# SEU-dynamical-models/Manifold-based-optical-flow-method

Measured on AMD Instinct MI355X. Metric: flow timesteps/sec on 160k-vertex mesh, higher is better.
Workload: dtype f32

## Files before the change

include/mof.h:

```cpp
#ifndef MOF_H_
#define MOF_H_

#include <stdint.h>

#ifdef __cplusplus
extern "C" {
#endif

#define MOF_ABI_VERSION 4

#define MOF_OK 0
#define MOF_E_ARG (-1)
#define MOF_E_HIP (-2)
#define MOF_E_NOCONV (-3)
#define MOF_E_STATE (-4)

#define MOF_GEOM_F32_POINTS 1u
#define MOF_NO_REORDER 2u

#define MOF_PREC_F64 0
#define MOF_PREC_MIXED 1

#define MOF_IO_DEVICE 1u
#define MOF_NO_BLOCK_JACOBI 2u
// ... 136 lines not shown

int mof_residual_probe(const int32_t *tri, int32_t N, int32_t M, uint32_t flags, int64_t *staged_bytes,
                       int32_t *staged_used);
int mof_test_force_residual_rows(int32_t on);
int mof_test_force_residual_trips(int32_t on);
int mof_test_residual_launches(int64_t *counts);

int mof_assembly_probe(const int32_t *tri, int32_t N, int32_t M, uint32_t flags, int64_t *staged_bytes,
                       int32_t *staged_used);
int mof_test_force_assembly_rows(int32_t on);
int mof_test_force_assembly_trips(int32_t on);
int mof_test_assembly_launches(int64_t *counts);
int mof_test_assembly_readback(mof_mesh *mesh, int32_t system, float *A32, void *A0h, double *rhs,
                               int32_t *have_A0h);

int mof_xcd_map_check(int32_t nblk, int32_t batch, int32_t group);
int mof_xcd_batch_cap(int64_t nblk, int32_t group, int32_t *batch);

typedef struct mof_dd mof_dd;

typedef struct mof_dd_info {
    int32_t nparts;
    int32_t local_parts;
    int32_t rank;
    int32_t max_neighbours;
    int32_t max_owned;
    int32_t pad_;
    int64_t ghost_rows;
    int64_t send_rows;
    double ms_setup;
// ... 45 lines not shown
```

manifold-based-optical-flow-method_amd/csrc/mof_abi.cpp:

```cpp
#include <algorithm>
#include <chrono>
#include <cmath>
#include <cstring>
#include <cstdio>
#include <cstdlib>
#include <functional>
#include <future>
#include <memory>
#include <mutex>
#include <new>

#include "mof_amg.h"
#include "mof_dd.h"
#include "mof_hostio.h"
#include "mof_internal.h"

namespace {

thread_local std::string g_err;

template <class F>
int guarded(F &&f) {
    try {
        f();
// ... 338 lines not shown
}

}

int mof_io_guard(const std::function<void()> &f) { return guarded(f); }

namespace mof {

std::atomic<int> g_force_index32{0};
std::atomic<int> g_force_residual_rows{0};
std::atomic<int> g_force_residual_trips{0};
std::atomic<int64_t> g_residual_launches[3];
std::atomic<int> g_force_assembly_rows{0};
std::atomic<int> g_force_assembly_trips{0};
std::atomic<int64_t> g_assembly_launches[3];

void raise_lds_limit(LdsLimit &st, int device, std::initializer_list<const void *> kernels, int64_t cap) {
    MOF_REQUIRE(device >= 0 && device < LdsLimit::kMaxDev, "device index out of range");
    std::call_once(st.once[device], [&] {
        for (const void *k : kernels)
            MOF_HIP(hipFuncSetAttribute(k, hipFuncAttributeMaxDynamicSharedMemorySize, (int)cap));
    });
}

void mesh_set_own(mof_mesh *m, int32_t nown) {
    MOF_HIP(hipSetDevice(m->device));
    m->n_own = nown;
    const int sym = knob(Knob::SymReads) ? (knob_int(Knob::SymReads, 0) != 0) : -1;
    std::shared_ptr<const MirrorTable> mt;
    {
// ... 13 lines not shown
        }
    }
    m->sym_reads = mt->used;
    const std::vector<int32_t> &mir = mt->table;
    m->sell_mir.alloc(mir.size());
    m->sell_mir.upload(mir.data(), mir.size(), m->stream);
    m->idx_packed = !mt->packed.empty() && !g_force_index32.load();
    if (m->idx_packed) {
        m->sell_idx.alloc(mt->packed.size());
        m->sell_idx.upload(mt->packed.data(), mt->packed.size(), m->stream);
    }
    m->res_lds_bytes = res_staged_bytes(m->pat);
    m->res_lds = m->res_lds_bytes <= kResLdsCap && !g_force_residual_rows.load();
    m->asm_lds_bytes = asm_staged_bytes(m->pat);
    m->asm_lds = asm_staged_fits(m->pat) && !g_force_assembly_rows.load();
    int64_t own = 0;
    for (int32_t v : mir) own += v >= 0 && !(v & kMirT);
    m->blocks_read = own;
    MOF_HIP(hipStreamSynchronize(m->stream));
}

constexpr int32_t kRowsPerWindow = 256;

void mesh_prepare_host(mof_mesh *m, const double *xyz, const double *nrm, const int32_t *tri,
                       const double *area, int32_t N, int32_t M, uint32_t flags, const int32_t *perm_in,
                       const int32_t *tri_ids) {
    m->N = N;
    m->n_own = N;
    m->M = M;
    m->flags = flags;
// ... 784 lines not shown
        MOF_REQUIRE(system >= 0 && system < w.JB && w.A32.n >= 4 * nb * (b + 1) &&
                        w.rhs.n >= 2 * (size_t)m->N * (b + 1),
                    "no mixed-precision assembly of that system in the workspace");
        MOF_HIP(hipStreamSynchronize(m->stream));
        if (A32) MOF_HIP(hipMemcpy(A32, w.A32.p + 4 * nb * b, 4 * nb * sizeof(float), hipMemcpyDeviceToHost));
        if (rhs)
            MOF_HIP(hipMemcpy(rhs, w.rhs.p + 2 * (size_t)m->N * b, 2 * (size_t)m->N * sizeof(double),
                              hipMemcpyDeviceToHost));
        const void *h = m->amg ? mof::amg_fine(m).A0h : nullptr;
        if (have_A0h) *have_A0h = h != nullptr;
        if (A0h && h)
            MOF_HIP(hipMemcpy(A0h, static_cast<const uint2 *>(h) + nb * b, nb * sizeof(uint2), hipMemcpyDeviceToHost));
    });
}

int mof_xcd_map_check(int32_t nblk, int32_t batch, int32_t group) {
    return guarded([&] {
        MOF_REQUIRE(nblk > 0 && batch > 0 && group >= 0, "bad arguments");
        MOF_REQUIRE(mof::xcd_map_covers(nblk, batch, group), "XCD order does not cover every (row block, system) once");
    });
}

int mof_xcd_batch_cap(int64_t nblk, int32_t group, int32_t *batch) {
    return guarded([&] {
        MOF_REQUIRE(nblk > 0 && group >= 0 && batch, "bad arguments");
        *batch = mof::xcd_batch_cap_host(nblk, group);
    });
}

int mof_bench_spmv(mof_mesh *m, uint32_t precision, int32_t batch, int32_t reps,
// ... 12 lines not shown
```

manifold-based-optical-flow-method_amd/csrc/mof_amg.hip:

```cpp
#include <algorithm>
#include <cstdio>
#include <cstdlib>

#include "mof_amg.h"
#include "mof_rowkern.h"

namespace mof {
namespace {

constexpr int kB3 = 12;

__device__ __forceinline__ bool retired(const int32_t *sysi, int32_t b) {
    return !sysi[b * kSysStride + SI_ACTIVE] || sysi[b * kSysStride + SI_CONV] >= 0;
}

template <int BS>
__device__ __forceinline__ void ldv(const float *v, int64_t node, float (&x)[BS]) {
    if constexpr (BS == 2) {
        const float2 t = reinterpret_cast<const float2 *>(v)[node];
        x[0] = t.x; x[1] = t.y;
    } else {
        const float4 t = reinterpret_cast<const float4 *>(v)[node];
        x[0] = t.x; x[1] = t.y; x[2] = t.z;
    }
// ... 64 lines not shown

__device__ __forceinline__ void st3(float *A, int64_t idx, const float (&a)[3][3]) {
    float4 *p = reinterpret_cast<float4 *>(A) + 3 * idx;
#pragma unroll
    for (int r = 0; r < 3; ++r) p[r] = make_float4(a[r][0], a[r][1], a[r][2], 0.f);
}

__device__ __forceinline__ void st_h9(uint4 *H, uint16_t *H22, int64_t q, const float (&c)[3][3]) {
    H[q] = make_uint4(bf16_bits(c[0][0]) | (bf16_bits(c[0][1]) << 16), bf16_bits(c[0][2]) | (bf16_bits(c[1][0]) << 16),
                      bf16_bits(c[1][1]) | (bf16_bits(c[1][2]) << 16), bf16_bits(c[2][0]) | (bf16_bits(c[2][1]) << 16));
    H22[q] = (uint16_t)bf16_bits(c[2][2]);
}

constexpr size_t kAhWords = 2, kAh22Words = 2;

__device__ __forceinline__ void st_a9(uint4 *H, uint16_t *H22, int64_t q, const float (&c)[3][3]) {
    {
        float m = 0.f;
#pragma unroll
        for (int r = 0; r < 3; ++r)
#pragma unroll
            for (int k = 0; k < 3; ++k) m = fmaxf(m, fabsf(c[r][k]));
        const uint32_t sb = bf16_bits(m / 127.f);
        const float sc = bf16_lo(sb);
        uint32_t u[9];
#pragma unroll
        for (int r = 0; r < 3; ++r)
#pragma unroll
            for (int k = 0; k < 3; ++k) {
                const float v = sc > 0.f ? rintf(c[r][k] / sc) : 0.f;
                u[3 * r + k] = (uint32_t)(fminf(fmaxf(v, -127.f), 127.f) + 128.f);
            }
        reinterpret_cast<uint2 *>(H)[q] =
            make_uint2(u[0] | (u[1] << 8) | (u[2] << 16) | (u[3] << 24), u[4] | (u[5] << 8) | (u[6] << 16) | (u[7] << 24));
        reinterpret_cast<uint32_t *>(H22)[q] = u[8] | (sb << 16);
    }
}
__device__ __forceinline__ void st_pair(float *__restrict__ Ac, uint4 *__restrict__ Ah, uint16_t *__restrict__ Ah22,
                                        int64_t b, int64_t c_sell_nb, int64_t pos, int32_t tw,
                                        const float (&C)[3][3]) {
    st3(Ac, b * c_sell_nb + pos, C);
    if (Ah) st_a9(Ah, Ah22, b * c_sell_nb + pos, C);
    if (tw >= 0) {
        float T[3][3];
#pragma unroll
        for (int r = 0; r < 3; ++r)
#pragma unroll
            for (int c = 0; c < 3; ++c) T[r][c] = C[c][r];
        st3(Ac, b * c_sell_nb + tw, T);
        if (Ah) st_a9(Ah, Ah22, b * c_sell_nb + tw, T);
    }
}


__global__ __launch_bounds__(kWG) void k_to_h0(int64_t n, const float4 *__restrict__ A, uint2 *__restrict__ H) {
    const int64_t q = (int64_t)blockIdx.x * kWG + threadIdx.x;
    if (q >= n) return;
    const float4 v = A[q];
    h0_st(H, q, v.x, v.y, v.z, v.w);
}

constexpr int kGalNS = 4;
__global__ __launch_bounds__(kWG) void k_galerkin0_ns(
    int64_t c_sell_nb, int32_t nC, int32_t B, const int32_t *__restrict__ c_sell_row,
    const int32_t *__restrict__ c_diag, const uint8_t *__restrict__ c_dead, const int32_t *__restrict__ c_twin,
// ... 73 lines not shown
    }
#pragma unroll
    for (int t = 0; t < kGalNS; ++t) {
        const int32_t b = b0 + t;
        if (b >= B) continue;
        if (pos == c_diag[I]) {
#pragma unroll
            for (int d = 0; d < 3; ++d)
                if (c_dead[3 * (int64_t)I + d]) Cm[t][d][d] += 1.f;
            float D[3][3];
            inv3(Cm[t], D);
            st_h9(Dh, Dh22, (int64_t)b * nC + I, D);
        }
        st_pair(Ac, Ah, Ah22, b, c_sell_nb, pos, c_twin[pos], Cm[t]);
    }
}

constexpr int kGalENS = 2;
__global__ __launch_bounds__(kWG) void k_galerkin0_ent(
    int32_t ngrp, const int32_t *__restrict__ ggrp, int32_t nC, int32_t B, const int32_t *__restrict__ c_sell_row,
    const int32_t *__restrict__ c_diag, const uint8_t *__restrict__ c_dead, const int32_t *__restrict__ c_twin, const int32_t *__restrict__ gptr,
    const int32_t *__restrict__ gent, const float *__restrict__ Q, const uint2 *__restrict__ Afh,
    int64_t f_sell_nb, int64_t c_sell_nb, float *__restrict__ Ac, uint4 *__restrict__ Dh,
    uint16_t *__restrict__ Dh22, uint4 *__restrict__ Ah, uint16_t *__restrict__ Ah22) {
#pragma clang fp contract(off)
    __shared__ float con[kGalENS][9][kWG];
    int32_t g, bq;
    const int32_t nq = (B + kGalENS - 1) / kGalENS;
    if (!xcd_map(ngrp, nq, g, bq, kGrpGal)) return;
    const int32_t b0 = bq * kGalENS;
// ... 6 lines not shown
        const int32_t pos = p0 + (int32_t)threadIdx.x / kGalENS;
        tI = c_sell_row[pos];
        tq0 = gptr[pos];
        tq1 = gptr[pos + 1];
        if (tI < nC) tdg = c_diag[tI];
    }
    if (e < e1) {
        const int32_t fp = gent[3 * (int64_t)e], ii = gent[3 * (int64_t)e + 1], jj = gent[3 * (int64_t)e + 2];
        float qi[6], qj[6], a[kGalENS][4];
#pragma unroll
        for (int k = 0; k < 6; ++k) {
            qi[k] = Q[(int64_t)ii * 6 + k];
            qj[k] = Q[(int64_t)jj * 6 + k];
        }
        const int32_t fq = fp < 0 ? 0 : fp & kMirPos;
        const bool tr = fp >= 0 && (fp & kMirT);
#pragma unroll
        for (int t = 0; t < kGalENS; ++t) {
            const int64_t bb = min(b0 + t, B - 1);
            h0_dec(h0_ld(Afh, bb * f_sell_nb + fq), a[t][0], a[t][1], a[t][2], a[t][3]);
            if (tr) {
                const float t01 = a[t][1];
                a[t][1] = a[t][2];
                a[t][2] = t01;
            }
            if (fp < 0) {
                const float d = fp == -1 ? 1.f : 0.f;
                a[t][0] = d; a[t][1] = 0.f; a[t][2] = 0.f; a[t][3] = d;
            }
        }
#pragma unroll
        for (int t = 0; t < kGalENS; ++t) {
            float T[2][3];
#pragma unroll
            for (int r = 0; r < 2; ++r)
#pragma unroll
                for (int c = 0; c < 3; ++c) T[r][c] = 1.f * (a[t][2 * r] * qj[c] + a[t][2 * r + 1] * qj[3 + c]);
#pragma unroll
            for (int r = 0; r < 3; ++r)
#pragma unroll
                for (int c = 0; c < 3; ++c) con[t][3 * r + c][threadIdx.x] = qi[r] * T[0][c] + qi[3 + r] * T[1][c];
        }
    }
    __syncthreads();
    for (int32_t task = threadIdx.x; task < np * kGalENS; task += kWG) {
        const int32_t pos = p0 + task / kGalENS, t = task % kGalENS, b = b0 + t;
        const bool first = task == (int32_t)threadIdx.x;
        const int32_t I = first ? tI : c_sell_row[pos];
        if (I >= nC || b >= B) continue;
        float Cm[3][3] = {};
        const int32_t q0 = first ? tq0 : gptr[pos], q1 = first ? tq1 : gptr[pos + 1];
        const bool diag = pos == (first ? tdg : c_diag[I]);
        if (q0 == q1 && !diag) continue;
        for (int32_t q = q0; q < q1; ++q)
#pragma unroll
            for (int k = 0; k < 9; ++k) Cm[k / 3][k % 3] += con[t][k][q - e0];
        if (diag) {
#pragma unroll
            for (int d = 0; d < 3; ++d)
                if (c_dead[3 * (int64_t)I + d]) Cm[d][d] += 1.f;
            float D[3][3];
            inv3(Cm, D);
            st_h9(Dh, Dh22, (int64_t)b * nC + I, D);
        }
        st_pair(Ac, Ah, Ah22, b, c_sell_nb, pos, c_twin[pos], Cm);
    }
}

constexpr int kSlab = 64;
constexpr int kSlabPos = 64;
template <typename T>
__global__ __launch_bounds__(kWG) void k_a_slab(int64_t f_sell_nb, int32_t b0, int32_t nb,
                                                const T *__restrict__ Af, T *__restrict__ AI) {
    __shared__ T t[kSlabPos][kSlab + 1];
    const int64_t q0 = (int64_t)blockIdx.x * kSlabPos;
    const int32_t lane = (int32_t)threadIdx.x & 63, w = (int32_t)threadIdx.x >> 6;
    for (int32_t s = w; s < kSlab; s += kWG / 64) {
        const int64_t q = q0 + lane;
        T v = {};
        if (s < nb && q < f_sell_nb) v = Af[(int64_t)(b0 + s) * f_sell_nb + q];
// ... 1590 lines not shown
    G.bf16_fresh = true;
    return AmgBf16{reinterpret_cast<uint2 *>(G.A0h.p)};
}

AmgFine amg_fine(mof_mesh *m) {
    AmgDevice &G = *m->amg;
    AmgFine f;
    f.A0h = G.A0h.p;
    f.sell_nb = m->pat.sell_nb();
    f.sell_off = m->sell_off.p;
    f.x0 = G.lv[0].x.p;
    f.omega = G.omega;
    f.smoothed = G.lv[0].smoothed;
    f.regular = G.regular;
    return f;
}

static uint4 *ah(AmgDevLevel &C) { return C.Ah.n > 1 ? reinterpret_cast<uint4 *>(C.Ah.p) : nullptr; }
static uint16_t *ah22(AmgDevLevel &C) { return C.Ah22.n > 1 ? C.Ah22.p : nullptr; }
static uint4 *dh(AmgDevLevel &C) { return reinterpret_cast<uint4 *>(C.Dh.p); }

void amg_setup_batch(mof_mesh *m, int32_t B, hipStream_t s) {
    AmgDevice &G = *m->amg;
    Workspace &w = m->ws;
    const size_t L = G.lv.size();
    if (!G.bf16_fresh) {
        const int64_t nb0 = m->pat.sell_nb() * B;
        k_to_h0<<<dim3((unsigned)((nb0 + kWG - 1) / kWG)), kWG, 0, s>>>(
            nb0, reinterpret_cast<const float4 *>(w.A32.p), reinterpret_cast<uint2 *>(G.A0h.p));
    }
// ... 36 lines not shown
                k_galerkin_sys<2><<<sys_grid(C.sell_nb), kWG, 0, s>>>(
                    C.sell_nb, C.n, B, b0, C.sell_row.p, C.diag_pos.p, C.dead.p, C.twin.p, F.gptr.p, F.gent.p, F.Q.p,
                    reinterpret_cast<const float4 *>(G.aslab.p), C.A.p, dh(C), C.Dh22.p, ah(C), ah22(C), cs);
            if (l1) {
                AmgDevLevel &C2 = G.lv[2];
                k_galerkin_sys<3><<<sys_grid(C2.sell_nb), kWG, 0, s>>>(
                    C2.sell_nb, C2.n, B, b0, C2.sell_row.p, C2.diag_pos.p, C2.dead.p, C2.twin.p, C.gptr.p, C.gent.p, C.Q.p,
                    reinterpret_cast<const float4 *>(C.slab.p), C2.A.p, dh(C2), C2.Dh22.p, ah(C2), ah22(C2), nullptr);
            }
        }
        l_first = l1 ? 2 : 1;
    }
    for (size_t l = l_first; l + 1 < L; ++l) {
        AmgDevLevel &F = G.lv[l], &C = G.lv[l + 1];
        const bool ent = ent_fits(F);
        if (l == 0 && ent)
            k_galerkin0_ent<<<dim3(xcd_grid(F.nggrp, (B + kGalENS - 1) / kGalENS, kGrpGal)), kWG, 0, s>>>(
                F.nggrp, F.ggrp.p, C.n, B, C.sell_row.p, C.diag_pos.p, C.dead.p, C.twin.p, F.gptr.p, F.gent.p, F.Q.p,
                reinterpret_cast<const uint2 *>(G.A0h.p), m->pat.sell_nb(), C.sell_nb, C.A.p, dh(C), C.Dh22.p, ah(C),
                ah22(C));
        else if (l == 0)
            k_galerkin0_ns<<<dim3(xcd_grid((int32_t)((C.sell_nb + kWG - 1) / kWG), (B + kGalNS - 1) / kGalNS,
                                           kGrpGal)),
                             kWG, 0, s>>>(C.sell_nb, C.n, B, C.sell_row.p, C.diag_pos.p, C.dead.p, C.twin.p, F.gptr.p, F.gent.p,
                                          F.Q.p, w.A32.p, m->pat.sell_nb(), C.A.p, dh(C), C.Dh22.p, ah(C), ah22(C),
                                          F.smoothed ? nullptr : reinterpret_cast<const uint2 *>(G.A0h.p));
        else if (ent) {
            if (F.nggrp > 0)
                k_galerkin3_ent<<<dim3(xcd_grid(F.nggrp, (B + kGalENS - 1) / kGalENS, kGrpGal)), kWG, 0, s>>>(
                    F.nggrp, F.ggrp.p, C.n, B, C.sell_row.p, C.diag_pos.p, C.dead.p, C.twin.p, F.gptr.p, F.gent.p, F.Q.p, F.A.p,
                    F.sell_nb, C.sell_nb, C.A.p, dh(C), C.Dh22.p, ah(C), ah22(C));
            if (F.nbig > 0)
                k_galerkin3_big<kGalBigNS>
                    <<<dim3(xcd_grid(F.nbig, (B + kGalBigNS - 1) / kGalBigNS, kGrpGal)), kWG, 0, s>>>(
                        F.nbig, F.gbig.p, C.n, B, C.sell_row.p, C.diag_pos.p, C.dead.p, C.twin.p, F.gptr.p, F.gent.p, F.Q.p,
                        F.A.p, F.sell_nb, C.sell_nb, C.A.p, dh(C), C.Dh22.p, ah(C), ah22(C));
        } else
            k_galerkin3_ns<kGal3NS>
                <<<dim3(xcd_grid((int32_t)((C.sell_nb + kWG - 1) / kWG), (B + kGal3NS - 1) / kGal3NS, kGrpGal)), kWG,
                   0, s>>>(C.sell_nb, C.n, B, C.sell_row.p, C.diag_pos.p, C.dead.p, C.twin.p, F.gptr.p, F.gent.p, F.Q.p, F.A.p,
                           F.sell_nb, C.A.p, dh(C), C.Dh22.p, ah(C), ah22(C));
    }
// ... 155 lines not shown
```

manifold-based-optical-flow-method_amd/csrc/mof_internal.h:

```cpp
#pragma once

#include <hip/hip_runtime.h>

#include <atomic>
#include <cstdint>
#include <cstdlib>
#include <functional>
#include <future>
#include <initializer_list>
#include <memory>
#include <mutex>
#include <string>
#include <type_traits>
#include <vector>

#include "../../include/mof.h"
#include "mof_knobs.h"

namespace mof {

constexpr int kWG = 256;
constexpr int kSlice = 64;

struct Error {
// ... 83 lines not shown
extern std::atomic<int> g_force_residual_rows;
extern std::atomic<int> g_force_residual_trips;
extern std::atomic<int64_t> g_residual_launches[3];
constexpr int64_t kAsmLdsCap = 160 * 1024;
constexpr int32_t kAsmLdsMaxW = 8;
inline int64_t asm_slice_bytes(int32_t w_a2, int32_t w_inc) {
    return (int64_t)kSlice * ((int64_t)w_inc * 112 + (int64_t)w_a2 * 48 + 48);
}
int64_t asm_staged_bytes(const Pattern &pat);
inline bool asm_staged_fits(const Pattern &pat) {
    return pat.max_w <= kAsmLdsMaxW && asm_staged_bytes(pat) <= kAsmLdsCap;
}
extern std::atomic<int> g_force_assembly_rows;
extern std::atomic<int> g_force_assembly_trips;
extern std::atomic<int64_t> g_assembly_launches[3];

struct LdsLimit {
    static constexpr int kMaxDev = 64;
    std::once_flag once[kMaxDev];
};
void raise_lds_limit(LdsLimit &st, int device, std::initializer_list<const void *> kernels, int64_t cap);

struct Workspace {
    int32_t cap = 0;
    int32_t nblk = 0;
    DevArray<double> u64, fc;
    DevArray<float> u32;
    DevArray<float> A32;
    DevArray<double> A64;
    DevArray<double> dinv64;
// ... 69 lines not shown
    std::vector<int32_t> agg_order;
    mof::DevArray<int32_t> perm_d;
    mof::DevArray<int32_t> tri_orig;
    mof::DevArray<int32_t> icol;
    mof::DevArray<int32_t> tri, vptr, vcol, cptr, clist, sell_off, sell_col, sell_blk, blk_row,
        diag_pos, tsell_off, tinc, tslot;
    mof::DevArray<int32_t> sell_mir;
    int64_t blocks_read = 0;
    bool sym_reads = false;
    mof::DevArray<uint32_t> sell_idx;
    bool idx_packed = false;
    int64_t res_lds_bytes = 0;
    bool res_lds = false;
    int64_t asm_lds_bytes = 0;
    bool asm_lds = false;
    mof::DevArray<double> e, gw, iw, area, a2;
    mof::DevArray<double> a2s64, w12_64;
    mof::DevArray<float> a2s32, w12_32;
    double a2s_lambda = 0.0;
    bool a2s_valid = false;
    mof::DevArray<double> Aexp, fexp;
    mof::Workspace ws;
    bool have_last_A = false;
    double ms_geometry = 0.0, ms_pattern = 0.0;
    int32_t *h_sysi = nullptr;
    double *h_sysd = nullptr;
    int32_t h_cap = 0;
    std::vector<hipEvent_t> spmv_events;
    std::vector<int32_t> iter_hint;
    mof::AmgDevice *amg = nullptr;
// ... 82 lines not shown
bool amg_build(mof_mesh *m);
void amg_ensure(mof_mesh *m, int32_t B);
void amg_setup_batch(mof_mesh *m, int32_t B, hipStream_t s);
void amg_vcycle(mof_mesh *m, int32_t B, const float *r, float *z, double *part_slot, int32_t nblk,
                const RedArgs &rd, hipStream_t s, bool zh, const int32_t *smap = nullptr, int32_t nl = 0);
struct AmgFine {
    const void *A0h;
    int64_t sell_nb;
    const int32_t *sell_off;
    float *x0;
    float omega;
    bool smoothed;
    bool regular;
};
AmgFine amg_fine(mof_mesh *m);
struct AmgBf16 {
    uint2 *A0h;
};
AmgBf16 amg_bf16_targets(mof_mesh *m, int32_t B);
void amg_destroy(AmgDevice *g);

int32_t amg_levels(const mof_mesh *m);
float amg_set_omega(mof_mesh *m, float omega);

bool xcd_map_covers(int32_t nblk, int32_t B, int32_t grp);
int32_t xcd_batch_cap_host(int64_t nblk, int32_t grp);
double bench_spmv(mof_mesh *m, uint32_t precision, int32_t B, int32_t reps, hipStream_t s,
                  double *bytes);

}
// ... 1 lines not shown
```

manifold-based-optical-flow-method_amd/mofhip/_lib.py:

```python
from __future__ import annotations

import ctypes
import os
import subprocess
import threading

import numpy as np

PKG_DIR = os.path.dirname(os.path.abspath(__file__))
ROOT_DIR = os.path.dirname(PKG_DIR)
CSRC_DIR = os.path.join(ROOT_DIR, "csrc")
LIB_PATH = os.environ.get("MOFHIP_LIB") or os.path.join(PKG_DIR, "libmofhip.so")

MOF_ABI_VERSION = 4

MOF_OK = 0
MOF_E_ARG = -1
MOF_E_HIP = -2
MOF_E_NOCONV = -3
MOF_E_STATE = -4

MOF_GEOM_F32_POINTS = 1
MOF_NO_REORDER = 2
MOF_PREC_F64 = 0
# ... 14 lines not shown

EXPORTS = (
    "mof_version", "mof_abi_version", "mof_last_error", "mof_device_count", "mof_mesh_create", "mof_mesh_clone",
    "mof_mesh_destroy", "mof_mesh_get_info", "mof_geometry_export", "mof_csr_export",
    "mof_assemble", "mof_solve_range", "mof_bench_spmv", "mof_velocity_vectors",
    "mof_csv_write", "mof_csv_shape", "mof_csv_read", "mof_ply_info", "mof_ply_read",
    "mof_point_normals", "mof_cell_areas", "mof_singularities", "mof_amg_probe",
    "mof_partition_rcb", "mof_dd_plan_info", "mof_dd_create", "mof_dd_unique_id",
    "mof_dd_create_rank", "mof_dd_destroy", "mof_dd_get_info", "mof_dd_solve_range",
    "mof_dd_test_fail_recovery_alloc", "mof_mesh_prepare", "mof_mesh_sync",
    "mof_singularities_compact", "mof_xcd_map_check", "mof_xcd_batch_cap", "mof_dd_create_rank_host",
    "mof_index_probe", "mof_test_force_index32", "mof_wave_speed", "mof_streamline_map", "mof_streamlines",
    "mof_test_streamline_pass", "mof_residual_probe", "mof_test_force_residual_rows",
    "mof_test_force_residual_trips", "mof_test_residual_launches", "mof_assembly_probe",
    "mof_test_force_assembly_rows", "mof_test_force_assembly_trips", "mof_test_assembly_launches",
    "mof_test_assembly_readback",
)


class MofError(RuntimeError):

    def __init__(self, code, msg):
        super().__init__("libmofhip error %d: %s" % (code, msg))
        self.code = code


class NotConverged(MofError):
    pass


class MofOpts(ctypes.Structure):
# ... 108 lines not shown
            "mof_test_streamline_pass": ([i32], ctypes.c_int),
            "mof_singularities": ([i32, P, P, i32, i32, P, i32, f64, u32, P, P, P, P, P],
                                  ctypes.c_int),
            "mof_amg_probe": ([P, P, i32, i32, P, P, P, P], ctypes.c_int),
            "mof_index_probe": ([P, i32, i32, u32, i32, P, P, P, P, P, P, P], ctypes.c_int),
            "mof_test_force_index32": ([i32], ctypes.c_int),
            "mof_residual_probe": ([P, i32, i32, u32, P, P], ctypes.c_int),
            "mof_test_force_residual_rows": ([i32], ctypes.c_int),
            "mof_test_force_residual_trips": ([i32], ctypes.c_int),
            "mof_test_residual_launches": ([P], ctypes.c_int),
            "mof_assembly_probe": ([P, i32, i32, u32, P, P], ctypes.c_int),
            "mof_test_force_assembly_rows": ([i32], ctypes.c_int),
            "mof_test_force_assembly_trips": ([i32], ctypes.c_int),
            "mof_test_assembly_launches": ([P], ctypes.c_int),
            "mof_test_assembly_readback": ([P, i32, P, P, P, P], ctypes.c_int),
            "mof_xcd_map_check": ([i32, i32, i32], ctypes.c_int),
            "mof_xcd_batch_cap": ([i64, i32, P], ctypes.c_int),
            "mof_singularities_compact": ([i32, P, P, i32, i32, P, i32, f64, u32, P, i64, P, P, P, P, P,
                                           P, P], ctypes.c_int),
            "mof_partition_rcb": ([P, i32, i32, P], ctypes.c_int),
            "mof_dd_plan_info": ([P, i32, i32, i32, P, P, P, P, P, P], ctypes.c_int),
            "mof_dd_create": ([P, P, P, P, i32, i32, i32, P, i32, u32, P], ctypes.c_int),
            "mof_dd_unique_id": ([P], ctypes.c_int),
            "mof_dd_create_rank": ([P, P, P, P, i32, i32, i32, P, i32, P, i32, u32, P],
                                   ctypes.c_int),
            "mof_dd_create_rank_host": ([P, P, P, P, i32, i32, i32, P, i32, P, i32, u32, P],
                                        ctypes.c_int),
            "mof_dd_destroy": ([P], ctypes.c_int),
            "mof_dd_get_info": ([P, P], ctypes.c_int),
            "mof_mesh_prepare": ([P, P], ctypes.c_int),
# ... 41 lines not shown
```

manifold-based-optical-flow-method_amd/mofhip/mesh.py:

```python
from __future__ import annotations

import ctypes
import threading
import time

import numpy as np

from . import _lib as L


def _f64(a):
    return np.ascontiguousarray(a, dtype=np.float64)


class DeviceMesh:

    def __init__(self, coordinates, normals, triangles, areas, device: int = 0,
                 reorder: bool = True):
        coords = np.asarray(coordinates)
        tri = np.asarray(triangles)
        if coords.ndim != 2 or coords.shape[1] != 3:
            raise ValueError("coordinates must be (N, 3)")
        if tri.ndim != 2 or tri.shape[1] != 3:
            raise ValueError("triangles must be (M, 3)")
# ... 328 lines not shown
    c = np.zeros(3, dtype=np.int64)
    L.check(L.lib().mof_test_assembly_launches(L.ptr(c)))
    return {"rows": int(c[0]), "staged_one": int(c[1]), "staged_multi": int(c[2])}


def assembly_readback(mesh: "DeviceMesh", system: int, device=None) -> dict:
    nb = int(mesh.info(device)["sell_blocks"])
    A32 = np.zeros((nb, 4), dtype=np.float32)
    A0h = np.zeros(nb, dtype=np.uint64)
    rhs = np.zeros((mesh.N, 2), dtype=np.float64)
    have = ctypes.c_int32(0)
    with mesh.lock(device):
        L.check(L.lib().mof_test_assembly_readback(mesh.handle(device), int(system), L.ptr(A32), L.ptr(A0h),
                                                   L.ptr(rhs), ctypes.byref(have)))
    return {"A32": A32, "A0h": A0h if have.value else None, "rhs": rhs}
```

Before: 4245.

## Stage Galerkin level-0 entry data in LDS and reuse across multiple systems

Adds a new level-0 Galerkin product kernel for unsmoothed hierarchies. Each workgroup stages its group's entry metadata and Q rows in LDS once, then each wavefront loops over several systems (trips) with wave-level barriers, reusing the staged data. It also reuses the quantized codes of a block for its transposed twin instead of re-quantizing. The cost is extra LDS use, wave-level sync subtleties and a new dispatch path, plus test hooks and a readback API.

New measurement: 4274 (median of 2 runs). About the same (+0.7%).

```diff
diff --git a/include/mof.h b/include/mof.h
--- a/include/mof.h
+++ b/include/mof.h
@@ -174,6 +174,12 @@
 int mof_test_assembly_readback(mof_mesh *mesh, int32_t system, float *A32, void *A0h, double *rhs,
                                int32_t *have_A0h);
 
+int mof_test_force_galerkin_entry(int32_t on);
+int mof_test_force_galerkin_trips(int32_t on);
+int mof_test_galerkin_launches(int64_t *counts);
+int mof_test_galerkin_readback(mof_mesh *mesh, int32_t system, int64_t *dims, float *A, void *Ah, void *Ah22,
+                               void *Dh, void *Dh22);
+
 int mof_xcd_map_check(int32_t nblk, int32_t batch, int32_t group);
 int mof_xcd_batch_cap(int64_t nblk, int32_t group, int32_t *batch);
 
diff --git a/manifold-based-optical-flow-method_amd/csrc/mof_abi.cpp b/manifold-based-optical-flow-method_amd/csrc/mof_abi.cpp
--- a/manifold-based-optical-flow-method_amd/csrc/mof_abi.cpp
+++ b/manifold-based-optical-flow-method_amd/csrc/mof_abi.cpp
@@ -376,6 +376,9 @@
 std::atomic<int> g_force_assembly_rows{0};
 std::atomic<int> g_force_assembly_trips{0};
 std::atomic<int64_t> g_assembly_launches[3];
+std::atomic<int> g_force_galerkin_entry{0};
+std::atomic<int> g_force_galerkin_trips{0};
+std::atomic<int64_t> g_galerkin_launches[4];
 
 void raise_lds_limit(LdsLimit &st, int device, std::initializer_list<const void *> kernels, int64_t cap) {
     MOF_REQUIRE(device >= 0 && device < LdsLimit::kMaxDev, "device index out of range");
@@ -419,6 +422,7 @@
     m->res_lds = m->res_lds_bytes <= kResLdsCap && !g_force_residual_rows.load();
     m->asm_lds_bytes = asm_staged_bytes(m->pat);
     m->asm_lds = asm_staged_fits(m->pat) && !g_force_assembly_rows.load();
+    m->gal_force_entry = g_force_galerkin_entry.load() != 0;
     int64_t own = 0;
     for (int32_t v : mir) own += v >= 0 && !(v & kMirT);
     m->blocks_read = own;
@@ -1233,6 +1237,31 @@
     });
 }
 
+int mof_test_force_galerkin_entry(int32_t on) {
+    return guarded([&] { mof::g_force_galerkin_entry.store(on != 0); });
+}
+
+int mof_test_force_galerkin_trips(int32_t on) {
+    return guarded([&] { mof::g_force_galerkin_trips.store(on != 0); });
+}
+
+int mof_test_galerkin_launches(int64_t *counts) {
+    return guarded([&] {
+        MOF_REQUIRE(counts, "NULL argument");
+        for (int k = 0; k < 4; ++k) counts[k] = mof::g_galerkin_launches[k].load();
+    });
+}
+
+int mof_test_galerkin_readback(mof_mesh *m, int32_t system, int64_t *dims, float *A, void *Ah, void *Ah22, void *Dh,
+                               void *Dh22) {
+    return guarded([&] {
+        MOF_REQUIRE(m, "mesh is NULL");
+        DeviceGuard dg(m->device);
+        mof::mesh_join_prep(m);
+        mof::amg_level1_readback(m, system, dims, A, Ah, Ah22, Dh, Dh22);
+    });
+}
+
 int mof_xcd_map_check(int32_t nblk, int32_t batch, int32_t group) {
     return guarded([&] {
         MOF_REQUIRE(nblk > 0 && batch > 0 && group >= 0, "bad arguments");
diff --git a/manifold-based-optical-flow-method_amd/csrc/mof_amg.hip b/manifold-based-optical-flow-method_amd/csrc/mof_amg.hip
--- a/manifold-based-optical-flow-method_amd/csrc/mof_amg.hip
+++ b/manifold-based-optical-flow-method_amd/csrc/mof_amg.hip
@@ -102,27 +102,31 @@
 
 constexpr size_t kAhWords = 2, kAh22Words = 2;
 
+__device__ __forceinline__ void a9_codes(const float (&c)[3][3], uint32_t (&u)[9], uint32_t &sb) {
+    float m = 0.f;
+#pragma unroll
+    for (int r = 0; r < 3; ++r)
+#pragma unroll
+        for (int k = 0; k < 3; ++k) m = fmaxf(m, fabsf(c[r][k]));
+    sb = bf16_bits(m / 127.f);
+    const float sc = bf16_lo(sb);
+#pragma unroll
+    for (int r = 0; r < 3; ++r)
+#pragma unroll
+        for (int k = 0; k < 3; ++k) {
+            const float v = sc > 0.f ? rintf(c[r][k] / sc) : 0.f;
+            u[3 * r + k] = (uint32_t)(fminf(fmaxf(v, -127.f), 127.f) + 128.f);
+        }
+}
+__device__ __forceinline__ void a9_put(uint4 *H, uint16_t *H22, int64_t q, const uint32_t (&u)[9], uint32_t sb) {
+    reinterpret_cast<uint2 *>(H)[q] =
+        make_uint2(u[0] | (u[1] << 8) | (u[2] << 16) | (u[3] << 24), u[4] | (u[5] << 8) | (u[6] << 16) | (u[7] << 24));
+    reinterpret_cast<uint32_t *>(H22)[q] = u[8] | (sb << 16);
+}
 __device__ __forceinline__ void st_a9(uint4 *H, uint16_t *H22, int64_t q, const float (&c)[3][3]) {
-    {
-        float m = 0.f;
-#pragma unroll
-        for (int r = 0; r < 3; ++r)
-#pragma unroll
-            for (int k = 0; k < 3; ++k) m = fmaxf(m, fabsf(c[r][k]));
-        const uint32_t sb = bf16_bits(m / 127.f);
-        const float sc = bf16_lo(sb);
-        uint32_t u[9];
-#pragma unroll
-        for (int r = 0; r < 3; ++r)
-#pragma unroll
-            for (int k = 0; k < 3; ++k) {
-                const float v = sc > 0.f ? rintf(c[r][k] / sc) : 0.f;
-                u[3 * r + k] = (uint32_t)(fminf(fmaxf(v, -127.f), 127.f) + 128.f);
-            }
-        reinterpret_cast<uint2 *>(H)[q] =
-            make_uint2(u[0] | (u[1] << 8) | (u[2] << 16) | (u[3] << 24), u[4] | (u[5] << 8) | (u[6] << 16) | (u[7] << 24));
-        reinterpret_cast<uint32_t *>(H22)[q] = u[8] | (sb << 16);
-    }
+    uint32_t u[9], sb;
+    a9_codes(c, u, sb);
+    a9_put(H, H22, q, u, sb);
 }
 __device__ __forceinline__ void st_pair(float *__restrict__ Ac, uint4 *__restrict__ Ah, uint16_t *__restrict__ Ah22,
                                         int64_t b, int64_t c_sell_nb, int64_t pos, int32_t tw,
@@ -137,6 +141,29 @@
             for (int c = 0; c < 3; ++c) T[r][c] = C[c][r];
         st3(Ac, b * c_sell_nb + tw, T);
         if (Ah) st_a9(Ah, Ah22, b * c_sell_nb + tw, T);
+    }
+}
+
+__device__ __forceinline__ void st_pair_t(float *__restrict__ Ac, uint4 *__restrict__ Ah, uint16_t *__restrict__ Ah22,
+                                          int64_t b, int64_t c_sell_nb, int64_t pos, int32_t tw,
+                                          const float (&C)[3][3]) {
+    uint32_t u[9] = {}, sb = 0;
+    st3(Ac, b * c_sell_nb + pos, C);
+    if (Ah) {
+        a9_codes(C, u, sb);
+        a9_put(Ah, Ah22, b * c_sell_nb + pos, u, sb);
+    }
+    if (tw >= 0) {
+        float T[3][3];
+#pragma unroll
+        for (int r = 0; r < 3; ++r)
+#pragma unroll
+            for (int c = 0; c < 3; ++c) T[r][c] = C[c][r];
+        st3(Ac, b * c_sell_nb + tw, T);
+        if (Ah) {
+            const uint32_t ut[9] = {u[0], u[3], u[6], u[1], u[4], u[7], u[2], u[5], u[8]};
+            a9_put(Ah, Ah22, b * c_sell_nb + tw, ut, sb);
+        }
     }
 }
 
@@ -240,6 +267,32 @@
         }
         st_pair(Ac, Ah, Ah22, b, c_sell_nb, pos, c_twin[pos], Cm[t]);
     }
+}
+
+__device__ __forceinline__ void gal0_block(uint2 h, int32_t fp, float (&a)[4]) {
+    h0_dec(h, a[0], a[1], a[2], a[3]);
+    if (fp >= 0 && (fp & kMirT)) {
+        const float t01 = a[1];
+        a[1] = a[2];
+        a[2] = t01;
+    }
+    if (fp < 0) {
+        const float d = fp == -1 ? 1.f : 0.f;
+        a[0] = d; a[1] = 0.f; a[2] = 0.f; a[3] = d;
+    }
+}
+__device__ __forceinline__ void gal0_term(const float (&a)[4], const float (&qi)[6], const float (&qj)[6],
+                                          float (&o)[9]) {
+#pragma clang fp contract(off)
+    float T[2][3];
+#pragma unroll
+    for (int r = 0; r < 2; ++r)
+#pragma unroll
+        for (int c = 0; c < 3; ++c) T[r][c] = 1.f * (a[2 * r] * qj[c] + a[2 * r + 1] * qj[3 + c]);
+#pragma unroll
+    for (int r = 0; r < 3; ++r)
+#pragma unroll
+        for (int c = 0; c < 3; ++c) o[3 * r + c] = qi[r] * T[0][c] + qi[3 + r] * T[1][c];
 }
 
 constexpr int kGalENS = 2;
@@ -276,32 +329,17 @@
             qj[k] = Q[(int64_t)jj * 6 + k];
         }
         const int32_t fq = fp < 0 ? 0 : fp & kMirPos;
-        const bool tr = fp >= 0 && (fp & kMirT);
 #pragma unroll
         for (int t = 0; t < kGalENS; ++t) {
             const int64_t bb = min(b0 + t, B - 1);
-            h0_dec(h0_ld(Afh, bb * f_sell_nb + fq), a[t][0], a[t][1], a[t][2], a[t][3]);
-            if (tr) {
-                const float t01 = a[t][1];
-                a[t][1] = a[t][2];
-                a[t][2] = t01;
-            }
-            if (fp < 0) {
-                const float d = fp == -1 ? 1.f : 0.f;
-                a[t][0] = d; a[t][1] = 0.f; a[t][2] = 0.f; a[t][3] = d;
-            }
+            gal0_block(h0_ld(Afh, bb * f_sell_nb + fq), fp, a[t]);
         }
 #pragma unroll
         for (int t = 0; t < kGalENS; ++t) {
-            float T[2][3];
-#pragma unroll
-            for (int r = 0; r < 2; ++r)
-#pragma unroll
-                for (int c = 0; c < 3; ++c) T[r][c] = 1.f * (a[t][2 * r] * qj[c] + a[t][2 * r + 1] * qj[3 + c]);
-#pragma unroll
-            for (int r = 0; r < 3; ++r)
-#pragma unroll
-                for (int c = 0; c < 3; ++c) con[t][3 * r + c][threadIdx.x] = qi[r] * T[0][c] + qi[3 + r] * T[1][c];
+            float o[9];
+            gal0_term(a[t], qi, qj, o);
+#pragma unroll
+            for (int k = 0; k < 9; ++k) con[t][k][threadIdx.x] = o[k];
         }
     }
     __syncthreads();
@@ -326,6 +364,164 @@
             st_h9(Dh, Dh22, (int64_t)b * nC + I, D);
         }
         st_pair(Ac, Ah, Ah22, b, c_sell_nb, pos, c_twin[pos], Cm);
+    }
+}
+
+#ifndef MOF_GAL_LDS_W
+#define MOF_GAL_LDS_W 4
+#endif
+#ifndef MOF_GAL_LDS_TRIPS
+#define MOF_GAL_LDS_TRIPS 4
+#endif
+#ifndef MOF_GAL_LDS_FILL
+#define MOF_GAL_LDS_FILL 2048
+#endif
+#ifndef MOF_GAL_LDS_GRP
+#define MOF_GAL_LDS_GRP 1
+#endif
+#ifndef MOF_GAL_LDS_PREFETCH
+#define MOF_GAL_LDS_PREFETCH 0
+#endif
+#ifndef MOF_GAL_LDS_TWIN
+#define MOF_GAL_LDS_TWIN 1
+#endif
+#ifndef MOF_GAL_LDS_ALIAS
+#define MOF_GAL_LDS_ALIAS 1
+#endif
+constexpr int kGalLdsW = MOF_GAL_LDS_W, kGalLdsTrips = MOF_GAL_LDS_TRIPS;
+constexpr int32_t kGrpGalLds = MOF_GAL_LDS_GRP;
+constexpr int64_t kGalLdsFill = MOF_GAL_LDS_FILL;
+constexpr int kGalLdsE = kWG / 64;
+#ifdef MOF_GAL_LDS_WPE
+#define MOF_GAL_LDS_ATTR __attribute__((amdgpu_waves_per_eu(MOF_GAL_LDS_WPE)))
+#else
+#define MOF_GAL_LDS_ATTR
+#endif
+template <int W>
+__global__ __launch_bounds__(64 * W) MOF_GAL_LDS_ATTR void k_galerkin0_lds(
+    int32_t ngrp, const int32_t *__restrict__ ggrp, int32_t nC, int32_t B, int32_t trips,
+    const int32_t *__restrict__ c_sell_row, const int32_t *__restrict__ c_diag, const uint8_t *__restrict__ c_dead,
+    const int32_t *__restrict__ c_twin, const int32_t *__restrict__ gptr, const int32_t *__restrict__ gent,
+    const float *__restrict__ Q, const uint2 *__restrict__ Afh, int64_t f_sell_nb, int64_t c_sell_nb,
+    float *__restrict__ Ac, uint4 *__restrict__ Dh, uint16_t *__restrict__ Dh22, uint4 *__restrict__ Ah,
+    uint16_t *__restrict__ Ah22) {
+#pragma clang fp contract(off)
+    constexpr int NT = 64 * W, E = kGalLdsE;
+    __shared__ int4 s_pos[kWG];
+    __shared__ float s_con[W][9][kWG];
+#if MOF_GAL_LDS_ALIAS
+    static_assert(13 <= 9 * W, "the entry stage does not fit the term scratch");
+    int32_t *const s_fp = reinterpret_cast<int32_t *>(&s_con[0][0][0]);
+    float(*const s_q)[kWG] = reinterpret_cast<float(*)[kWG]>(&s_con[0][0][0]) + 1;
+#else
+    __shared__ int32_t s_fp[kWG];
+    __shared__ float s_q[12][kWG];
+#endif
+    int32_t g, chunk;
+    const int32_t PW = W * trips;
+    if (!xcd_map(ngrp, (B + PW - 1) / PW, g, chunk, kGrpGalLds)) return;
+    const int32_t wv = __builtin_amdgcn_readfirstlane(threadIdx.x >> 6), l = threadIdx.x & 63;
+    const int32_t p0 = ggrp[2 * g], p1 = ggrp[2 * g + 1];
+    const int32_t e0 = gptr[p0], ne = gptr[p1] - e0, np = p1 - p0;
+    for (int32_t t = threadIdx.x; t < ne; t += NT) {
+        const int64_t e = (int64_t)e0 + t;
+        const int32_t fp = gent[3 * e], ii = gent[3 * e + 1], jj = gent[3 * e + 2];
+        s_fp[t] = fp;
+#pragma unroll
+        for (int k = 0; k < 6; ++k) {
+            s_q[k][t] = Q[(int64_t)ii * 6 + k];
+            s_q[6 + k][t] = Q[(int64_t)jj * 6 + k];
+        }
+    }
+    for (int32_t t = threadIdx.x; t < np; t += NT) {
+        const int32_t pos = p0 + t, I = c_sell_row[pos];
+        const int32_t q0 = gptr[pos] - e0, q1 = gptr[pos + 1] - e0;
+        int4 r = make_int4(-1, q0 | (q1 << 16), c_twin[pos], 0);
+        if (I < nC) {
+            const bool diag = pos == c_diag[I];
+            if (q0 != q1 || diag) r.x = I;
+            if (diag)
+                r.w = 1 | (c_dead[3 * (int64_t)I] ? 2 : 0) | (c_dead[3 * (int64_t)I + 1] ? 4 : 0) |
+                      (c_dead[3 * (int64_t)I + 2] ? 8 : 0);
+        }
+        s_pos[t] = r;
+    }
+    __syncthreads();
+    float qi[E][6], qj[E][6];
+    int32_t fp[E];
+#pragma unroll
+    for (int u = 0; u < E; ++u) {
+        const int32_t t = min(l + 64 * u, max(ne - 1, 0));
+        fp[u] = s_fp[t];
+#pragma unroll
+        for (int k = 0; k < 6; ++k) {
+            qi[u][k] = s_q[k][t];
+            qj[u][k] = s_q[6 + k][t];
+        }
+    }
+#if MOF_GAL_LDS_ALIAS
+    __syncthreads();
+#endif
+    float(*con)[kWG] = s_con[wv];
+    auto load = [&](int32_t b, uint2(&h)[E]) {
+        const uint2 *Ab = Afh + (int64_t)b * f_sell_nb;
+#pragma unroll
+        for (int u = 0; u < E; ++u)
+            if (l + 64 * u < ne) h[u] = h0_ld(Ab, fp[u] < 0 ? 0 : fp[u] & kMirPos);
+    };
+    int32_t b = chunk * PW + wv;
+    if (b >= B) return;
+    uint2 h[E] = {};
+    load(b, h);
+#pragma unroll 1
+    for (int32_t trip = 0;; ++trip) {
+        const int32_t bn = b + W;
+        const bool more = trip + 1 < trips && bn < B;
+        uint2 hn[E] = {};
+        if (MOF_GAL_LDS_PREFETCH && more) load(bn, hn);
+#pragma unroll
+        for (int u = 0; u < E; ++u)
+            if (l + 64 * u < ne) {
+                float a[4], o[9];
+                gal0_block(h[u], fp[u], a);
+                gal0_term(a, qi[u], qj[u], o);
+#pragma unroll
+                for (int k = 0; k < 9; ++k) con[k][l + 64 * u] = o[k];
+            }
+        __builtin_amdgcn_fence(__ATOMIC_RELEASE, "wavefront");
+        __builtin_amdgcn_wave_barrier();
+        __builtin_amdgcn_fence(__ATOMIC_ACQUIRE, "wavefront");
+        for (int32_t t = l; t < np; t += 64) {
+            const int4 r = s_pos[t];
+            const int32_t I = r.x;
+            if (I < 0) continue;
+            const int32_t q0 = r.y & 0xFFFF, q1 = r.y >> 16;
+            float Cm[3][3] = {};
+            for (int32_t q = q0; q < q1; ++q)
+#pragma unroll
+                for (int k = 0; k < 9; ++k) Cm[k / 3][k % 3] += con[k][q];
+            if (r.w & 1) {
+#pragma unroll
+                for (int d = 0; d < 3; ++d)
+                    if (r.w & (2 << d)) Cm[d][d] += 1.f;
+                float D[3][3];
+                inv3(Cm, D);
+                st_h9(Dh, Dh22, (int64_t)b * nC + I, D);
+            }
+#if MOF_GAL_LDS_TWIN
+            st_pair_t(Ac, Ah, Ah22, b, c_sell_nb, p0 + t, r.z, Cm);
+#else
+            st_pair(Ac, Ah, Ah22, b, c_sell_nb, p0 + t, r.z, Cm);
+#endif
+        }
+        if (!more) break;
+        __builtin_amdgcn_fence(__ATOMIC_RELEASE, "wavefront");
+        __builtin_amdgcn_wave_barrier();
+        __builtin_amdgcn_fence(__ATOMIC_ACQUIRE, "wavefront");
+        if (!MOF_GAL_LDS_PREFETCH) load(bn, hn);
+#pragma unroll
+        for (int u = 0; u < E; ++u) h[u] = hn[u];
+        b = bn;
     }
 }
 
@@ -1946,6 +2142,32 @@
     f.smoothed = G.lv[0].smoothed;
     f.regular = G.regular;
     return f;
+}
+
+void amg_level1_readback(mof_mesh *m, int32_t system, int64_t *dims, float *A, void *Ah, void *Ah22, void *Dh,
+                         void *Dh22) {
+    MOF_REQUIRE(m->amg && m->amg->lv.size() >= 2, "the handle has no multigrid hierarchy");
+    AmgDevice &G = *m->amg;
+    AmgDevLevel &C = G.lv[1];
+    const size_t nb = (size_t)C.sell_nb, n = (size_t)C.n, b = (size_t)system;
+    const bool have_ah = C.Ah.n > 1;
+    if (dims) {
+        dims[0] = C.sell_nb;
+        dims[1] = C.n;
+        dims[2] = have_ah;
+        dims[3] = G.lv[0].smoothed;
+    }
+    if (!A && !Ah && !Ah22 && !Dh && !Dh22) return;
+    MOF_REQUIRE(system >= 0 && system < G.cap && C.A.n >= kB3 * nb * (b + 1), "no product of that system on the handle");
+    MOF_HIP(hipStreamSynchronize(m->stream));
+    if (A) MOF_HIP(hipMemcpy(A, C.A.p + kB3 * nb * b, kB3 * nb * sizeof(float), hipMemcpyDeviceToHost));
+    if (Ah && have_ah)
+        MOF_HIP(hipMemcpy(Ah, C.Ah.p + kAhWords * nb * b, kAhWords * nb * sizeof(uint32_t), hipMemcpyDeviceToHost));
+    if (Ah22 && have_ah)
+        MOF_HIP(hipMemcpy(Ah22, C.Ah22.p + kAh22Words * nb * b, kAh22Words * nb * sizeof(uint16_t),
+                          hipMemcpyDeviceToHost));
+    if (Dh) MOF_HIP(hipMemcpy(Dh, C.Dh.p + 4 * n * b, 4 * n * sizeof(uint32_t), hipMemcpyDeviceToHost));
+    if (Dh22) MOF_HIP(hipMemcpy(Dh22, C.Dh22.p + n * b, n * sizeof(uint16_t), hipMemcpyDeviceToHost));
 }
 
 static uint4 *ah(AmgDevLevel &C) { return C.Ah.n > 1 ? reinterpret_cast<uint4 *>(C.Ah.p) : nullptr; }
@@ -2012,18 +2234,32 @@
     for (size_t l = l_first; l + 1 < L; ++l) {
         AmgDevLevel &F = G.lv[l], &C = G.lv[l + 1];
         const bool ent = ent_fits(F);
-        if (l == 0 && ent)
+        if (l == 0 && !F.smoothed && F.nggrp > 0 && !m->gal_force_entry) {
+            int32_t trips = kGalLdsTrips;
+            const bool one = (int64_t)F.nggrp * ((B + kGalLdsW * trips - 1) / (kGalLdsW * trips)) < kGalLdsFill &&
+                             !g_force_galerkin_trips.load();
+            if (one) trips = 1;
+            const unsigned grid = xcd_grid(F.nggrp, (B + kGalLdsW * trips - 1) / (kGalLdsW * trips), kGrpGalLds);
+            MOF_REQUIRE((int64_t)grid * 64 * kGalLdsW < ((int64_t)1 << 32), "launch grid past 2^32 work-items");
+            g_galerkin_launches[one ? 2 : 3]++;
+            k_galerkin0_lds<kGalLdsW><<<dim3(grid), 64 * kGalLdsW, 0, s>>>(
+                F.nggrp, F.ggrp.p, C.n, B, trips, C.sell_row.p, C.diag_pos.p, C.dead.p, C.twin.p, F.gptr.p, F.gent.p,
+                F.Q.p, reinterpret_cast<const uint2 *>(G.A0h.p), m->pat.sell_nb(), C.sell_nb, C.A.p, dh(C), C.Dh22.p,
+                ah(C), ah22(C));
+        } else if (l == 0 && ent) {
+            g_galerkin_launches[1]++;
             k_galerkin0_ent<<<dim3(xcd_grid(F.nggrp, (B + kGalENS - 1) / kGalENS, kGrpGal)), kWG, 0, s>>>(
                 F.nggrp, F.ggrp.p, C.n, B, C.sell_row.p, C.diag_pos.p, C.dead.p, C.twin.p, F.gptr.p, F.gent.p, F.Q.p,
                 reinterpret_cast<const uint2 *>(G.A0h.p), m->pat.sell_nb(), C.sell_nb, C.A.p, dh(C), C.Dh22.p, ah(C),
                 ah22(C));
-        else if (l == 0)
+        } else if (l == 0) {
+            g_galerkin_launches[0]++;
             k_galerkin0_ns<<<dim3(xcd_grid((int32_t)((C.sell_nb + kWG - 1) / kWG), (B + kGalNS - 1) / kGalNS,
                                            kGrpGal)),
                              kWG, 0, s>>>(C.sell_nb, C.n, B, C.sell_row.p, C.diag_pos.p, C.dead.p, C.twin.p, F.gptr.p, F.gent.p,
                                           F.Q.p, w.A32.p, m->pat.sell_nb(), C.A.p, dh(C), C.Dh22.p, ah(C), ah22(C),
                                           F.smoothed ? nullptr : reinterpret_cast<const uint2 *>(G.A0h.p));
-        else if (ent) {
+        } else if (ent) {
             if (F.nggrp > 0)
                 k_galerkin3_ent<<<dim3(xcd_grid(F.nggrp, (B + kGalENS - 1) / kGalENS, kGrpGal)), kWG, 0, s>>>(
                     F.nggrp, F.ggrp.p, C.n, B, C.sell_row.p, C.diag_pos.p, C.dead.p, C.twin.p, F.gptr.p, F.gent.p, F.Q.p, F.A.p,
diff --git a/manifold-based-optical-flow-method_amd/csrc/mof_internal.h b/manifold-based-optical-flow-method_amd/csrc/mof_internal.h
--- a/manifold-based-optical-flow-method_amd/csrc/mof_internal.h
+++ b/manifold-based-optical-flow-method_amd/csrc/mof_internal.h
@@ -121,6 +121,9 @@
 extern std::atomic<int> g_force_assembly_rows;
 extern std::atomic<int> g_force_assembly_trips;
 extern std::atomic<int64_t> g_assembly_launches[3];
+extern std::atomic<int> g_force_galerkin_entry;
+extern std::atomic<int> g_force_galerkin_trips;
+extern std::atomic<int64_t> g_galerkin_launches[4];
 
 struct LdsLimit {
     static constexpr int kMaxDev = 64;
@@ -220,6 +223,7 @@
     bool res_lds = false;
     int64_t asm_lds_bytes = 0;
     bool asm_lds = false;
+    bool gal_force_entry = false;
     mof::DevArray<double> e, gw, iw, area, a2;
     mof::DevArray<double> a2s64, w12_64;
     mof::DevArray<float> a2s32, w12_32;
@@ -332,6 +336,8 @@
     bool regular;
 };
 AmgFine amg_fine(mof_mesh *m);
+void amg_level1_readback(mof_mesh *m, int32_t system, int64_t *dims, float *A, void *Ah, void *Ah22, void *Dh,
+                         void *Dh22);
 struct AmgBf16 {
     uint2 *A0h;
 };
diff --git a/manifold-based-optical-flow-method_amd/mofhip/_lib.py b/manifold-based-optical-flow-method_amd/mofhip/_lib.py
--- a/manifold-based-optical-flow-method_amd/mofhip/_lib.py
+++ b/manifold-based-optical-flow-method_amd/mofhip/_lib.py
@@ -52,7 +52,8 @@
     "mof_test_streamline_pass", "mof_residual_probe", "mof_test_force_residual_rows",
     "mof_test_force_residual_trips", "mof_test_residual_launches", "mof_assembly_probe",
     "mof_test_force_assembly_rows", "mof_test_force_assembly_trips", "mof_test_assembly_launches",
-    "mof_test_assembly_readback",
+    "mof_test_assembly_readback", "mof_test_force_galerkin_entry", "mof_test_force_galerkin_trips",
+    "mof_test_galerkin_launches", "mof_test_galerkin_readback",
 )
 
 
@@ -191,6 +192,10 @@
             "mof_test_force_assembly_trips": ([i32], ctypes.c_int),
             "mof_test_assembly_launches": ([P], ctypes.c_int),
             "mof_test_assembly_readback": ([P, i32, P, P, P, P], ctypes.c_int),
+            "mof_test_force_galerkin_entry": ([i32], ctypes.c_int),
+            "mof_test_force_galerkin_trips": ([i32], ctypes.c_int),
+            "mof_test_galerkin_launches": ([P], ctypes.c_int),
+            "mof_test_galerkin_readback": ([P, i32, P, P, P, P, P, P], ctypes.c_int),
             "mof_xcd_map_check": ([i32, i32, i32], ctypes.c_int),
             "mof_xcd_batch_cap": ([i64, i32, P], ctypes.c_int),
             "mof_singularities_compact": ([i32, P, P, i32, i32, P, i32, f64, u32, P, i64, P, P, P, P, P,
diff --git a/manifold-based-optical-flow-method_amd/mofhip/mesh.py b/manifold-based-optical-flow-method_amd/mofhip/mesh.py
--- a/manifold-based-optical-flow-method_amd/mofhip/mesh.py
+++ b/manifold-based-optical-flow-method_amd/mofhip/mesh.py
@@ -366,3 +366,48 @@
         L.check(L.lib().mof_test_assembly_readback(mesh.handle(device), int(system), L.ptr(A32), L.ptr(A0h),
                                                    L.ptr(rhs), ctypes.byref(have)))
     return {"A32": A32, "A0h": A0h if have.value else None, "rhs": rhs}
+
+
+class force_galerkin_entry:
+
+    def __enter__(self):
+        L.check(L.lib().mof_test_force_galerkin_entry(1))
+        return self
+
+    def __exit__(self, *exc):
+        L.check(L.lib().mof_test_force_galerkin_entry(0))
+        return False
+
+
+class force_galerkin_trips:
+
+    def __enter__(self):
+        L.check(L.lib().mof_test_force_galerkin_trips(1))
+        return self
+
+    def __exit__(self, *exc):
+        L.check(L.lib().mof_test_force_galerkin_trips(0))
+        return False
+
+
+def galerkin_launches() -> dict:
+    c = np.zeros(4, dtype=np.int64)
+    L.check(L.lib().mof_test_galerkin_launches(L.ptr(c)))
+    return {"position": int(c[0]), "entry": int(c[1]), "staged_one": int(c[2]), "staged_multi": int(c[3])}
+
+
+def galerkin_readback(mesh: "DeviceMesh", system: int, device=None) -> dict:
+    dims = np.zeros(4, dtype=np.int64)
+    with mesh.lock(device):
+        h = mesh.handle(device)
+        L.check(L.lib().mof_test_galerkin_readback(h, int(system), L.ptr(dims), None, None, None, None, None))
+        nb, n, have = int(dims[0]), int(dims[1]), bool(dims[2])
+        A = np.zeros((nb, 12), dtype=np.float32)
+        Ah = np.zeros((nb, 2), dtype=np.uint32)
+        Ah22 = np.zeros((nb, 2), dtype=np.uint16)
+        Dh = np.zeros((n, 4), dtype=np.uint32)
+        Dh22 = np.zeros(n, dtype=np.uint16)
+        L.check(L.lib().mof_test_galerkin_readback(h, int(system), None, L.ptr(A), L.ptr(Ah), L.ptr(Ah22),
+                                                   L.ptr(Dh), L.ptr(Dh22)))
+    return {"A": A, "Ah": Ah if have else None, "Ah22": Ah22 if have else None, "Dh": Dh, "Dh22": Dh22,
+            "smoothed": bool(dims[3])}
```
